# QWTforGithub/CDSegNet

Measured on AMD Instinct MI355X. Metric: points/sec/node (ScanNet ~120k-pt scenes, 1-step), higher is better.
Workload: dtype f16

## Files before the change

### cdsegnet_amd/_lib.py

```python
import ctypes
import os
import threading
from ctypes import POINTER, Structure, c_char_p, c_float, c_int, c_int32, c_int64, c_long, c_size_t, c_uint64, c_void_p

HERE = os.path.dirname(os.path.abspath(__file__))
LIB_PATH = os.path.join(HERE, "libcdseg_hip.so")
LIB_PATH_F16 = os.path.join(HERE, "libcdseg_hip_f16.so")

F32, BF16 = 0, 1
ACT_NONE, ACT_GELU, ACT_SWISH = 0, 1, 2
ORDER_IDS = {"z": 0, "z-trans": 1, "hilbert": 2, "hilbert-trans": 3}
ERRORS = {-1: "CDSEG_ERR_ARG", -2: "CDSEG_ERR_LAUNCH", -3: "CDSEG_ERR_WORKSPACE", -4: "CDSEG_ERR_UNSUPPORTED"}


class CdsegError(RuntimeError):
    pass


class DuplicateVoxelsError(CdsegError):

    def __init__(self, msg, count):
        super().__init__(msg)
        self.count = int(count)

# ... 155 lines not shown
    "cdseg_attn_tail_rr": (c_int, [c_void_p, c_int, c_void_p, c_void_p, c_void_p, c_void_p, c_float, c_void_p, c_void_p,
                                   c_void_p, c_int, c_void_p, c_int, c_long, c_int, c_void_p]),
    "cdseg_cpe_head_rr2": (c_int, [c_void_p, c_int, c_void_p, c_void_p, c_void_p, c_void_p, c_void_p, c_int, c_void_p, c_int,
                                   c_void_p, c_void_p, c_void_p, c_float, c_void_p, c_void_p, c_int, c_long, c_int, c_int, c_void_p]),
    "cdseg_attn_tail_rr2": (c_int, [c_void_p, c_int, c_void_p, c_void_p, c_void_p, c_void_p, c_float, c_void_p, c_void_p,
                                    c_void_p, c_int, c_void_p, c_int, c_void_p, c_int, c_long, c_int, c_void_p, c_size_t, c_void_p]),
    "cdseg_block_scratch_bytes": (c_size_t, [POINTER(BlockDesc), c_long]),
    "cdseg_block_forward": (c_int, [POINTER(BlockDesc), POINTER(BlockIO), c_void_p]),
    "cdseg_layernorm": (c_int, [c_void_p, c_int, c_int, c_void_p, c_void_p, c_float, c_void_p, c_int, c_void_p,
                                c_void_p, c_int, c_int, c_void_p, c_int, c_int, c_long, c_int, c_void_p]),
    "cdseg_attention": (c_int, [c_void_p, c_void_p, c_void_p, c_int, c_int, c_int, c_void_p, c_void_p, c_void_p,
                                c_void_p, c_int, c_int, c_int, c_float, c_void_p, c_int, c_int, c_void_p]),
    "cdseg_attention_ex": (c_int, [c_void_p, c_void_p, c_void_p, c_int, c_int, c_int, c_void_p, c_void_p, c_void_p,
                                   c_void_p, c_int, c_int, c_int, c_float, c_void_p, c_int, c_int, c_int, c_void_p]),
    "cdseg_attention_schedule": (c_long, [c_int, c_int, c_int, c_int, c_void_p, c_long]),
    "cdseg_attention_bwd_ws_bytes": (c_size_t, [c_long, c_int]),
    "cdseg_attention_bwd": (c_int, [c_void_p, c_void_p, c_void_p, c_int, c_int, c_int, c_void_p, c_void_p, c_void_p, c_void_p,
                                    c_int, c_int, c_long, c_int, c_float, c_void_p, c_int, c_void_p, c_void_p, c_void_p,
                                    c_int, c_int, c_int, c_int, c_void_p, c_size_t, c_void_p]),
    "cdseg_layernorm_bwd": (c_int, [c_void_p, c_int, c_void_p, c_float, c_void_p, c_int, c_void_p, c_int, c_int, c_void_p,
                                    c_void_p, c_long, c_int, c_void_p]),
    "cdseg_gelu_bwd": (c_int, [c_void_p, c_void_p, c_void_p, c_long, c_void_p]),
    "cdseg_conv_wgrad": (c_int, [c_void_p, c_int, c_void_p, c_int, c_void_p, c_int, c_long, c_int, c_int, c_void_p, c_void_p,
                                 c_void_p]),
    "cdseg_linear_wgrad": (c_int, [c_void_p, c_int, c_void_p, c_void_p, c_int, c_long, c_int, c_int, c_void_p, c_int, c_void_p,
                                   c_void_p]),
    "cdseg_conv_wgrad16": (c_int, [c_void_p, c_int, c_void_p, c_int, c_void_p, c_int, c_long, c_int, c_int, c_void_p, c_void_p,
                                   c_void_p]),
    "cdseg_linear_wgrad16": (c_int, [c_void_p, c_int, c_void_p, c_void_p, c_int, c_long, c_int, c_int, c_void_p, c_int, c_void_p,
                                     c_void_p]),
# ... 99 lines not shown
```

### cdsegnet_amd/csrc/deep.h

```cpp
#pragma once
#include "common.h"

bool deep_supported(int channels);
int deep_pack(int channels, const void* wl, const void* wqkv, void* head_img, const void* wp, const void* w1, const void* w2,
              void* tail_img, hipStream_t s);
int deep_head(const void* y, int ldy, const void* head_img, const float* bl, const float* lnp_g, const float* lnp_b,
              const float* x, int ldx, float* x_out, int ldxo, const float* colbias, const float* ln1_g, const float* ln1_b,
              float eps, const float* bqkv, void* qkv, int ldqkv, long n, int channels, int qkv_flags, hipStream_t s,
              const float* ypart = nullptr, int ysplits = 1, const float* ybias = nullptr);
struct cdseg_gemm_args;
int gemm_leave_partials(const cdseg_gemm_args* a, int* splits, void* stream);
int deep_tail(const void* o, int ldo, const void* tail_img, const float* bp, const float* ln_g, const float* ln_b, float eps,
              const float* b1, const float* b2, const float* x_in, int ldxi, float* x, int ldx, void* xc, int ldxc, long n,
              int channels, void* ws, size_t ws_bytes, hipStream_t s);
```

### cdsegnet_amd/csrc/gemm.hip

```cpp
#include <cstdlib>

#include <atomic>

#include "common.h"
#include "prof.h"

#ifndef CDSEG_CONV_SQ128_MIN_M
#define CDSEG_CONV_SQ128_MIN_M 8000
#endif
#ifndef CDSEG_CONV_SQ128_MAX_M
#define CDSEG_CONV_SQ128_MAX_M 32768
#endif

namespace {

struct GemmP {
  const void* A;
  const void* W;
  const float* bias;
  const float* scale;
  const float* shift;
  const float* res;
  const float* add_src;
  const int32_t* add_idx;
// ... 11 lines not shown
  int splits;
  int kshift;
  long nbr_sm, nbr_so;
  int gm, gn;
  int xmode;
  int fix;
  const float* colbias;
  const float* ln_pre_g;
  const float* ln_pre_b;
  const float* ln_post_g;
  const float* ln_post_b;
  void* ln_out;
  int ldln, ln_out_dtype;
  float ln_eps;
  int alt;
#ifdef CDSEG_EXPERIMENTS
  int dbg;
#endif
};

struct F32X3 { float v; };
template <typename CT> constexpr bool kIsX3 = false;
template <> constexpr bool kIsX3<F32X3> = true;
typedef _Float16 x3_f16x2_t __attribute__((ext_vector_type(2)));
typedef _Float16 x3_f16x8_t __attribute__((ext_vector_type(8)));

__device__ __forceinline__ void x3_split2(float a, float b, uint32_t& hi, uint32_t& lo) {
  const hw_f32x2_t v = {__builtin_amdgcn_fmed3f(a, -65504.f, 65504.f), __builtin_amdgcn_fmed3f(b, -65504.f, 65504.f)};
  const x3_f16x2_t h = __builtin_convertvector(v, x3_f16x2_t);
  const hw_f32x2_t hf = __builtin_convertvector(h, hw_f32x2_t);
// ... 227 lines not shown
  }
  if (g.ln_post_g) {
    float4 h[MAXG];
    row_layernorm(g.ln_post_g, g.ln_post_b, h);
    if (act_row) {
#pragma unroll
      for (int i = 0; i < MAXG; ++i) {
        const int cg = part + L * i;
        if (cg < groups) store_vec4(g.ln_out, g.ln_out_dtype, m * g.ldln + c0 + 4 * cg, h[i]);
      }
    }
  }
}

__global__ void splitk_epilogue_kernel(GemmP g) {
  const long groups = g.M * (long)(g.N >> 2);
  const long t = (long)blockIdx.x * blockDim.x + threadIdx.x;
  if (t >= groups) return;
  const long m = t / (g.N >> 2);
  const int n = (int)(t - m * (g.N >> 2)) << 2;
  const long stride = g.M * (long)g.N;
  const float* p = g.ws + m * g.N + n;
  float4 v = *reinterpret_cast<const float4*>(p);
  for (int s = 1; s < g.splits; ++s) {
    const float4 u = *reinterpret_cast<const float4*>(p + s * stride);
    v.x += u.x; v.y += u.y; v.z += u.z; v.w += u.w;
  }
  epilogue4(g, m, n, v);
}

__global__ __launch_bounds__(256) void row_finish_kernel(GemmP g) {
  const int lane = threadIdx.x & 63;
  const long m = (long)blockIdx.x * 4 + (threadIdx.x >> 6);
  if (m >= g.M) return;
  const int groups = g.N >> 2;
  const long sstride = g.M * (long)g.N;
  float4 v[2];
#pragma unroll
  for (int i = 0; i < 2; ++i) {
    v[i] = make_float4(0.f, 0.f, 0.f, 0.f);
    if (lane + 64 * i < groups) {
      const float* p = g.ws + m * g.N + 4 * (lane + 64 * i);
      v[i] = *reinterpret_cast<const float4*>(p);
// ... 8 lines not shown

#ifdef CDSEG_GEMM_TIMING
__device__ unsigned long long g_gemm_t[8 * 16384];
extern "C" int cdseg_debug_gemm_timing(unsigned long long* host_dst, size_t count) {
  return hipMemcpyFromSymbol(host_dst, HIP_SYMBOL(g_gemm_t), count * sizeof(unsigned long long)) == hipSuccess ? 0 : -2;
}
__device__ unsigned long long g_gemm_kt[4096 * 16 * 8];
extern "C" int cdseg_debug_gemm_ktiming(unsigned long long* host_dst, size_t count) {
  return hipMemcpyFromSymbol(host_dst, HIP_SYMBOL(g_gemm_kt), count * sizeof(unsigned long long)) == hipSuccess ? 0 : -2;
}
#define KT_STAMP(x) const unsigned long long x = __builtin_readcyclecounter()
#else
#define KT_STAMP(x)
#endif

template <int BN, int BM, bool SQ = false, int AI = 2, int AJ = BN / 32>
__device__ __forceinline__ void tile_epilogue(const GemmP& g, f32x4_t (&acc)[AI][AJ], char* smem, int tid, int lane,
                                              int wm, int wn, long m0, int n0, int zs) {
  constexpr int NT = SQ ? 512 : 4 * BM;
  constexpr int TN = BN / 32;
  constexpr int CLD = BN + 4;
  const int fr = lane & 15, fg = lane >> 4;
  float* Cs = reinterpret_cast<float*>(smem);
  const bool plain = !g.fix && plain_bf16_out(g);
  Cols8 cols;
  if (plain) cols = load_cols8(g, n0 + 8 * (tid % (BN / 8)));
  auto lds_barrier = [] {
    asm volatile("s_waitcnt lgkmcnt(0)" ::: "memory");
    __builtin_amdgcn_s_barrier();
  };
#pragma unroll 1
  for (int hh = 0; hh < BM / 64; ++hh) {
#ifdef CDSEG_GEMM_TIMING
    if (tid == 0 && blockIdx.x < 16384) g_gemm_t[(size_t)blockIdx.x * 8 + 4 + 2 * hh] = __builtin_readcyclecounter();
#endif
    if (hh) lds_barrier();
    int zcol = 0;
    if constexpr (BM > 64) asm volatile("v_mov_b32 %0, 0" : "=v"(zcol));
    if constexpr (SQ) {
// ... 9 lines not shown
      const int rbase = (wm & 1) * 32;
#pragma unroll
      for (int i = 0; i < 2; ++i)
#pragma unroll
        for (int j = 0; j < TN; ++j)
#pragma unroll
          for (int r = 0; r < 4; ++r)
            Cs[(rbase + i * 16 + fg * 4 + r) * CLD + wn * (BN / 2) + j * 16 + fr] = acc[i][j][r];
    }
    lds_barrier();
#ifdef CDSEG_GEMM_TIMING
    if (tid == 0 && blockIdx.x < 16384) g_gemm_t[(size_t)blockIdx.x * 8 + 5 + 2 * hh] = __builtin_readcyclecounter();
#endif
    const long mb = m0 + 64 * hh;
    constexpr int GPR = BN / 4;
    if (g.fix) {
      for (int item = tid; item < 64 * GPR; item += NT) {
        const int row = item / GPR, cg = item % GPR;
        const long m = mb + row;
        const int n = n0 + 4 * cg;
        if (m >= g.M || n >= g.N) continue;
        *reinterpret_cast<float4*>(g.ws + ((long)zs * g.M + m) * g.N + n) =
            *reinterpret_cast<const float4*>(Cs + row * CLD + 4 * cg);
      }
    } else if (BM == 64 && (g.ln_pre_g || g.ln_post_g)) {
      constexpr int MAXG = BN / 16;
      const int row = (tid >> 2) & 63, part = tid & 3;
      const long m = mb + row;
      const int ng = g.N >> 2;
      float4 v[MAXG];
#pragma unroll
      for (int i = 0; i < MAXG; ++i)
        v[i] = (part + 4 * i < ng) ? *reinterpret_cast<const float4*>(Cs + row * CLD + 4 * (part + 4 * i))
                                   : make_float4(0.f, 0.f, 0.f, 0.f);
      finish_row<MAXG>(g, m, m < g.M, part, 4, ng, 0, v);
    } else if (plain) {
      static_assert(NT % (GPR / 2) == 0, "a lane's columns must not change between items");
// ... 259 lines not shown
    if (kc + 1 < kc1) store_tiles();
    __syncthreads();
  }

  if constexpr (kIsX3<CT>) {
#pragma unroll
    for (int i = 0; i < 2; ++i)
#pragma unroll
      for (int j = 0; j < TN; ++j) acc[i][j] += accx[i][j] * (1.0f / 2048.f);
  }
  tile_epilogue<BN, BM>(g, acc, smem, tid, lane, wm, wn, m0, n0, zs);
}

__device__ uint4 g_zero_page[8];

template <int BM, bool GATHER = true, int BN = 128, int NST = 2, bool SQ = false>
struct DmaCfg {
  static constexpr int WAVES = SQ ? 8 : BM / 16, NT = WAVES * 64, BK = 64;
  static constexpr int A_BYTES = BM * 128, W_BYTES = BN * 128;
  static constexpr int A_PW = (BM / 8) / WAVES, W_PW = (BN / 8) / WAVES;
  static constexpr int STAGES = NST * (A_BYTES + W_BYTES);
  static constexpr int ITAB = GATHER ? BM * 27 * 4 : 0;
  static constexpr int LDS = STAGES + ITAB + 1024;
};

template <int BM, bool GATHER, int BN = 128, int NST = 2, bool SQ = false>
__global__ __launch_bounds__(SQ ? 512 : 4 * BM) void gemm_dma_kernel(GemmP g) {
#ifdef CDSEG_GEMM_TIMING
  const unsigned long long rt0 = __builtin_amdgcn_s_memrealtime(), tc0 = __builtin_readcyclecounter();
#endif
  using D = DmaCfg<BM, GATHER, BN, NST, SQ>;
  constexpr int TN = BN / 32;
  constexpr int AI = SQ ? 4 : 2, AJ = TN;
  static_assert(!SQ || (BM == 256 && NST == 2 && GATHER), "SQ: 256-row tiles of 8 waves, two stages, sparse convs");
  extern __shared__ __attribute__((aligned(16))) char smem[];
  char* tail = smem + D::STAGES + D::ITAB;
  int* live = reinterpret_cast<int*>(tail);
  int* glive = reinterpret_cast<int*>(tail + 256);
  unsigned long long* smask = reinterpret_cast<unsigned long long*>(tail + 640);
  int* itab = reinterpret_cast<int*>(smem + D::STAGES);

  const int tid = threadIdx.x;
  const int lane = tid & 63;
  const int wave = __builtin_amdgcn_readfirstlane(tid >> 6);
  const int wm = wave >> 1, wn = wave & 1;
  int mt, sl;
  {
    const int bid = blockIdx.x, slices = g.gn * g.splits;
    if (g.xmode == 1) {
      const int j = bid >> 3;
      mt = j % g.gm;
      sl = (bid & 7) + 8 * (j / g.gm);
      if (sl >= slices) return;
    } else if (g.xmode == 2) {
      const int j = bid >> 3, chunk = (g.gm + 7) >> 3;
      mt = (bid & 7) * chunk + j / slices;
      sl = j % slices;
      if (j / slices >= chunk || mt >= g.gm) return;
    } else {
      mt = bid % g.gm;
      sl = bid / g.gm;
    }
  }
  const int nt = sl % g.gn, zs = sl / g.gn;
  const long m0 = (long)mt * BM;
  const int n0 = nt * BN;
  const long Kw = (long)g.kvol * g.K;

  int nlive = 1;
  if (GATHER) {
    constexpr int OPT = D::NT / BM, PASSES = (27 + OPT - 1) / OPT;
    int* glraw = reinterpret_cast<int*>(tail + 384);
    int* slotmap = reinterpret_cast<int*>(tail + 512);
    const int r = tid % BM, og = tid / BM;
    if (tid < 32) glraw[tid] = 0;
    __syncthreads();
    int idx[PASSES];
#pragma unroll
// ... 23 lines not shown
    __syncthreads();
    nlive = __builtin_amdgcn_readfirstlane(live[0]);
#pragma unroll
    for (int i = 0; i < PASSES; ++i) {
      const int o = og + OPT * i;
      if (o < g.kvol) {
        const int sl2 = slotmap[o];
        if (sl2 >= 0) itab[r * 27 + sl2] = idx[i];
      }
    }
    __syncthreads();
  }
  const int KV = nlive * g.K;
  const int nkc = KV / D::BK;
  const int kshift = g.kshift;
  const int kc0 = (int)(((long)nkc * zs) / g.splits);
  const int kc1 = (int)(((long)nkc * (zs + 1)) / g.splits);

  const int lrow = lane >> 3, slot = lane & 7;
  const bf16_t* a_src[D::A_PW];
  int a_row[D::A_PW];
  int a_chunk[D::A_PW];
  const bf16_t* w_src[D::W_PW];
  int w_chunk[D::W_PW];
#pragma unroll
  for (int i = 0; i < D::A_PW; ++i) {
    const int r = (wave * D::A_PW + i) * 8 + lrow;
    a_row[i] = r;
    a_chunk[i] = slot ^ ((r >> 1) & 7);
    long m = m0 + r;
    if (m >= g.M) m = g.M - 1;
    a_src[i] = (const bf16_t*)g.A + m * g.lda + a_chunk[i] * 8;
// ... 217 lines not shown
  }
#ifdef CDSEG_GEMM_TIMING
  if (lane == 0 && blockIdx.x < 4096 && wave < 16) {
    unsigned long long* d = g_gemm_kt + ((size_t)blockIdx.x * 16 + wave) * 8;
    d[0] = kt_wait; d[1] = kt_bar; d[2] = kt_issue; d[3] = kt_mma; d[4] = (unsigned long long)(kc1 - kc0); d[5] = kt_pro;
    d[6] = (unsigned long long)nlive; d[7] = 1;
  }
#endif
  __syncthreads();
#ifdef CDSEG_EXPERIMENTS
  if (g.dbg & 4) { if (acc[0][0][0] == 12345.678f) ((float*)g.out)[0] = acc[1][1][1]; return; }
#endif
#ifdef CDSEG_GEMM_TIMING
  const unsigned long long tc1 = __builtin_readcyclecounter();
#endif
  tile_epilogue<BN, BM, SQ, AI, AJ>(g, acc, smem, tid, lane, wm, wn, m0, n0, zs);
#ifdef CDSEG_GEMM_TIMING
  if (tid == 0 && blockIdx.x < 16384) {
    unsigned long long* d = g_gemm_t + (size_t)blockIdx.x * 8;
    d[0] = rt0; d[1] = __builtin_amdgcn_s_memrealtime(); d[2] = tc1 - tc0;
    const unsigned long long tend = __builtin_readcyclecounter();
    d[3] = tend - tc1;
    const unsigned long long a0 = d[4], a1 = d[5], b0 = d[6], b1 = d[7];
    d[4] = a1 - a0; d[5] = b0 - a1; d[6] = b1 - b0; d[7] = tend - b1;
  }
#endif
}

thread_local bool tl_leave_partials = false;
thread_local int tl_partial_splits = 1;

template <typename CT, int BN, int NCH, int BM>
constexpr int gemm_smem_bytes() {
  constexpr int ab = (BM + BN) * NCH * 16, c = 64 * (BN + 4) * 4;
  return (ab > c ? ab : c) + 1024;
}


template <typename CT, int NCH, bool GATHER>
int launch_bn(GemmP p, size_t ws_bytes, hipStream_t s) {
  constexpr int BK = NCH * (16 / (int)sizeof(CT));
  static const int split_target = cdseg_knob("CDSEG_GEMM_SPLIT_TARGET", 320);
  static const int split_max = cdseg_knob("CDSEG_GEMM_SPLIT_MAX", 16);
  static const int xmode_env = cdseg_knob("CDSEG_GEMM_XMODE", -1);
  const bool ln = p.ln_pre_g || p.ln_post_g;
// ... 10 lines not shown
  }
  int dma_use_bm = -1;
  if constexpr (NCH == 16 && sizeof(CT) == 2) {
    static const int dma_on0 = cdseg_knob("CDSEG_GEMM_DMA", 1);
    static const int dma_bm0 = cdseg_knob("CDSEG_GEMM_DMA_BM", 0);
    if (dma_on0 && p.N > 64 && (p.K % 64) == 0 && (!GATHER || (p.kshift >= 6 && p.kvol <= 27)) && p.M >= 128) {
      int want = dma_bm0 ? dma_bm0 : ((GATHER || p.M >= 16384 || (p.N >= 1024 && p.M >= 2048)) ? 128 : 64);
      if (ln && p.N <= 128) want = -1;
      if (want > 0) bm = dma_use_bm = want;
    }
  }
  bool sq = false;
  int sq_bn = 256;
  if constexpr (GATHER && NCH == 16 && sizeof(CT) == 2) {
    static const int sq_on = cdseg_knob("CDSEG_CONV_SQ", 1);
    static const int sq_min_m = cdseg_knob("CDSEG_CONV_SQ_MIN_M", 5000);
    static const int sq_min_n = cdseg_knob("CDSEG_CONV_SQ_MIN_N", 256);
    sq = sq_on && dma_use_bm == 128 && p.kvol == 27 && p.N >= sq_min_n && (p.N % 256) == 0 && !ln && p.kshift >= 6 &&
         p.M >= sq_min_m && p.ws && p.vec_ok && !p.out_idx;
    static const int sq128_min_m = cdseg_knob("CDSEG_CONV_SQ128_MIN_M", CDSEG_CONV_SQ128_MIN_M);
    static const int sq128_max_m = cdseg_knob("CDSEG_CONV_SQ128_MAX_M", CDSEG_CONV_SQ128_MAX_M);
    if (!sq && sq_on && sq128_min_m > 0 && dma_use_bm == 128 && p.kvol == 27 && p.N == 128 && !ln && p.kshift >= 6 &&
        p.M >= sq128_min_m && p.M < sq128_max_m && p.vec_ok && !p.out_idx) {
      sq = true;
      sq_bn = 128;
    }
    if (sq) {
      bm = 256;
      p.alt = cdseg_knob("CDSEG_CONV_SQ_ALT", 1);
    }
  }
  const int gm = (int)((p.M + bm - 1) / bm);
  bool wide = false;
  if constexpr (GATHER && NCH == 16 && sizeof(CT) == 2) {
    static const int wide_on = cdseg_knob("CDSEG_CONV_WIDE", 0);
    wide = !sq && wide_on && dma_use_bm == 128 && p.kvol == 27 && p.N >= 256 && (p.N % 256) == 0 && !ln;
  }
  const int bn = wide ? 256 : (sq ? sq_bn : (p.N <= 32 ? 32 : (p.N <= 64 ? 64 : 128)));
  const int gn = (p.N + bn - 1) / bn;
  int splits = 1;
  const long nkc = ((long)p.kvol * p.K + BK - 1) / BK;
  const long blocks = (long)gm * gn;
  const bool can_fix = p.ws && p.vec_ok && !p.out_idx;
  static const int plain_min_nkc = cdseg_knob("CDSEG_GEMM_SPLIT_MIN_NKC", 16);
  if (can_fix && blocks < 256 && nkc >= (GATHER ? 4 : plain_min_nkc)) {
    int smax = (int)(nkc / 2);
    if (smax > split_max) smax = split_max;
    while (smax > 1 && (size_t)smax * p.M * p.N * sizeof(float) > ws_bytes) --smax;
    if (wide || sq) {
      splits = (int)(256 / blocks);
    } else {
      splits = (int)((split_target + blocks - 1) / blocks);
    }
    if (splits > smax) splits = smax;
    if (!wide && !sq)
      for (int c = splits; c <= smax && c < splits + 4; ++c)
        if ((gn * c) % 8 == 0) { splits = c; break; }
    if (splits < 1) splits = 1;
  }
  p.fix = 0;
  if (splits > 1) p.fix = ln ? 2 : 1;
  else if (ln && gn > 1) p.fix = 2;
  if (p.fix) {
    if (!can_fix || (size_t)splits * p.M * p.N * sizeof(float) > ws_bytes) return CDSEG_ERR_WORKSPACE;
    if (p.fix == 2 && p.N > 512) return CDSEG_ERR_UNSUPPORTED;
  }
  p.splits = splits;
  p.gm = gm;
  p.gn = gn;
  const int slices = gn * splits;
  const long wbytes = (long)p.N * p.kvol * p.K * (long)sizeof(CT);
  p.xmode = 0;
  if (sq) p.xmode = gm >= 64 ? 2 : 0;
  else if (slices >= 8 && wbytes >= (1 << 20) && gm > 1) p.xmode = 1;
  else if (GATHER && gm >= 64) p.xmode = 2;
  if (xmode_env >= 0) p.xmode = (xmode_env == 1 && slices < 8) ? 0 : xmode_env;
  unsigned nblk;
  if (p.xmode == 1) nblk = 8u * (unsigned)((slices + 7) / 8) * (unsigned)gm;
  else if (p.xmode == 2) nblk = 8u * (unsigned)((gm + 7) / 8) * (unsigned)slices;
  else nblk = (unsigned)gm * (unsigned)slices;
  const dim3 grid(nblk);
  bool launched = false;
  if constexpr (NCH == 16 && sizeof(CT) == 2) {
    static const int dma_on = cdseg_knob("CDSEG_GEMM_DMA", 1);
    static const int dma_bm = cdseg_knob("CDSEG_GEMM_DMA_BM", 0);
    const bool fused_ln_here = ln && gn == 1 && splits == 1;
    if constexpr (GATHER) {
      if (sq && dma_on && sq_bn == 128) {
        launched = true;
        using Q = DmaCfg<256, true, 128, 2, true>;
        static std::atomic<bool> aq128{false};
        if (!aq128) {
          if (hipFuncSetAttribute((const void*)gemm_dma_kernel<256, true, 128, 2, true>, hipFuncAttributeMaxDynamicSharedMemorySize,
// ... 129 lines not shown
    else hipLaunchKernelGGL((gemm_kernel<CT, 128, NCH, GATHER>), grid, dim3(256), 0, s, p);
  }
  if (hipGetLastError() != hipSuccess) return CDSEG_ERR_LAUNCH;
  if (p.fix == 2) {
    hipLaunchKernelGGL(row_finish_kernel, dim3((unsigned)((p.M + 3) / 4)), dim3(256), 0, s, p);
    if (hipGetLastError() != hipSuccess) return CDSEG_ERR_LAUNCH;
  } else if (p.fix == 1) {
    if (tl_leave_partials && p.vec_ok && p.bias && !p.scale && p.act == CDSEG_ACT_NONE && !p.res && !p.add_src && !p.out2 &&
        !p.out_idx && !p.colbias) {
      tl_partial_splits = p.splits;
      return CDSEG_OK;
    }
    const long groups = p.M * (long)(p.N >> 2);
    hipLaunchKernelGGL(splitk_epilogue_kernel, dim3((unsigned)((groups + 255) / 256)), dim3(256), 0, s, p);
    if (hipGetLastError() != hipSuccess) return CDSEG_ERR_LAUNCH;
  }
  return CDSEG_OK;
}

template <typename CT, bool GATHER>
int launch(const GemmP& p, size_t ws_bytes, hipStream_t s) {
  const long ktot = (long)p.kvol * p.K;
  if (ktot <= 64) {
    if constexpr (sizeof(CT) == 2) return launch_bn<CT, 4, GATHER>(p, ws_bytes, s);
    else return launch_bn<CT, 8, GATHER>(p, ws_bytes, s);
  }
  return launch_bn<CT, 16, GATHER>(p, ws_bytes, s);
}

}
// ... 53 lines not shown
  if (a->compute_dtype == CDSEG_BF16) rc = a->nbr ? launch<bf16_t, true>(p, wsb, s) : launch<bf16_t, false>(p, wsb, s);
  else if (a->compute_dtype == CDSEG_F32) rc = a->nbr ? launch<float, true>(p, wsb, s) : launch<float, false>(p, wsb, s);
  else if (a->compute_dtype == CDSEG_F32X3) rc = a->nbr ? launch<F32X3, true>(p, wsb, s) : launch<F32X3, false>(p, wsb, s);
  if (prof) cdseg_prof_end(tok, s);
  return rc;
}

int gemm_leave_partials(const cdseg_gemm_args* a, int* splits, void* stream) {
  tl_leave_partials = true;
  tl_partial_splits = 1;
  const int rc = cdseg_gemm(a, stream);
  tl_leave_partials = false;
  *splits = tl_partial_splits;
  return rc;
}
```

### cdsegnet_amd/csrc/runtime.hip

```cpp
#include <cstdlib>
#include <cstring>

#include "common.h"
#include "deep.h"

namespace {

inline size_t align_up(size_t v, size_t a) { return (v + a - 1) / a * a; }

struct Carver {
  char* base;
  size_t off, cap;
  void* take(size_t bytes) {
    off = align_up(off, 256);
    void* p = base ? base + off : nullptr;
    off += bytes;
    return p;
  }
};

constexpr int FUSE_LN_MAX_C = 512;
constexpr size_t SPLITK_WS_CAP = (size_t)64 << 20;

inline size_t esz(int dtype) { return dtype == CDSEG_BF16 ? 2 : 4; }
inline int storage_dtype(int dtype) { return dtype == CDSEG_F32X3 ? CDSEG_F32 : dtype; }

struct Layout {
  void *y, *h, *qkv, *o, *u, *y2, *ws, *xs;
  size_t ws_bytes, total;
};

Layout carve(const cdseg_block_desc* d, long n, void* scratch) {
  Carver c{(char*)scratch, 0, 0};
  const size_t e = esz(d->dtype);
  const size_t C = d->channels;
  Layout L;
  L.y = c.take(n * C * e);
  L.h = c.take(n * C * e);
  L.qkv = c.take(n * 3 * C * e);
  L.o = c.take(n * C * e);
  L.u = c.take(n * (size_t)d->hidden * e);
  L.y2 = d->channels > FUSE_LN_MAX_C ? c.take(n * C * 4) : nullptr;
  const long tiles = ((n + 63) / 64) * (((long)C + 127) / 128);
  L.ws_bytes = tiles < 256 ? (size_t)32 * n * (size_t)(3 * C > (size_t)d->hidden ? 3 * C : d->hidden) * 4
                           : (C > 128 ? (size_t)n * C * 4 : 0);
  if (C >= 256 && ((n + 127) / 128) * (((long)C + 255) / 256) < 256) {
    const size_t want = (size_t)8 * n * C * 4;
    if (want > L.ws_bytes) L.ws_bytes = want;
  }
  if (L.ws_bytes > SPLITK_WS_CAP) L.ws_bytes = SPLITK_WS_CAP;
  L.ws = L.ws_bytes ? c.take(L.ws_bytes) : nullptr;
  L.xs = (d->dtype == CDSEG_BF16 && C >= 128 && d->head_img && d->tail_img) ? c.take(n * C * 4) : nullptr;
  L.total = align_up(c.off, 256);
  return L;
}

cdseg_gemm_args base_args(const cdseg_block_desc* d, const Layout& L, long n) {
  cdseg_gemm_args a;
  std::memset(&a, 0, sizeof(a));
  a.M = n;
  a.kvol = 1;
  a.a_dtype = storage_dtype(d->dtype);
  a.compute_dtype = d->dtype;
  a.ws = L.ws;
  a.ws_bytes = L.ws_bytes;
  a.ln_eps = d->ln_eps;
// ... 36 lines not shown
  int rc;
  int attn_flags = d->attn_flags & CDSEG_ATTN_Q_PRESCALED;

  const bool conv_fits = n * 27 * 4 < (1l << 31) && n * (long)C * 2 < (1l << 31) - 65536;
  const bool deep_head_next = cdseg_knob("CDSEG_DEEP_FUSED", 1) != 0 && T == CDSEG_BF16 && (C == 128 || C == 256) &&
                              d->hidden == 4 * C && d->head_img;
  int ysplits = 1;
  const float* ypart = nullptr;
  if (d->cpe_conv_wimg && T == CDSEG_BF16 && (C == 32 || C == 64) && conv_fits) {
    rc = cdseg_subm_conv3(io->xc_in, C, d->cpe_conv_wimg, (const float*)d->cpe_conv_b, io->nbr, n, C, L.y, C, stream);
    if (rc != CDSEG_OK) return rc;
  } else {
    cdseg_gemm_args a = base_args(d, L, n);
    a.A = io->xc_in; a.lda = C; a.W = d->cpe_conv_w; a.bias = d->cpe_conv_b; a.nbr = io->nbr; a.nbr_kmajor = 1; a.kvol = 27;
    a.N = C; a.K = C; a.out = L.y; a.ldo = C; a.out_dtype = T;
    static const bool partials_on = cdseg_knob("CDSEG_CONV_PARTIALS", 1) != 0;
    if (partials_on && deep_head_next && (C == 128 || C == 256) && !io->sat_counter && a.ws && a.bias) {
      if ((rc = gemm_leave_partials(&a, &ysplits, stream)) != CDSEG_OK) return rc;
      if (ysplits > 1) ypart = (const float*)a.ws;
    } else if ((rc = cdseg_gemm(&a, stream)) != CDSEG_OK) {
      return rc;
    }
  }
  static const bool fused_head = cdseg_knob("CDSEG_FUSED_HEAD", 1) != 0;
  static const bool deep_on = cdseg_knob("CDSEG_DEEP_FUSED", 1) != 0;
  static const long deep512_min = cdseg_knob("CDSEG_DEEP512_MIN_ROWS", CDSEG_DEEP512_MIN_ROWS);
  static const bool deep512_split = cdseg_knob("CDSEG_DEEP_SPLIT", 1) != 0;
  const bool deep = deep_on && T == CDSEG_BF16 &&
                    (C == 128 || C == 256 || (C == 512 && (n >= deep512_min || (deep512_split && L.xs)))) && d->hidden == 4 * C;
  const bool head = (fused_head && T == CDSEG_BF16 && (C == 32 || C == 64)) || (deep && d->head_img);
// ... 125 lines not shown
```

### cdsegnet_amd/ops.py

```python
import ctypes
import os
import threading

import torch

from . import _lib
from ._lib import ACT_GELU, ACT_NONE, ACT_SWISH, BF16, F32, GemmArgs, check

__all__ = ["ACT_NONE", "ACT_GELU", "ACT_SWISH", "F32", "BF16"]

LP_DTYPES = {"bf16": torch.bfloat16, "f16": torch.float16}


class _Dtypes:

    def __getitem__(self, dtype):
        if dtype == torch.float32:
            return F32
        if dtype == LP_DTYPES[_lib.active()]:
            return BF16
        raise _lib.CdsegError(f"{dtype} tensors do not belong to the active build of the library ({_lib.active()})")


_DT = _Dtypes()
# ... 504 lines not shown
        a.ln_pre_g, a.ln_pre_b = ln_pre[0].data_ptr(), ln_pre[1].data_ptr()
    else:
        a.ln_pre_g = a.ln_pre_b = None
    if ln_post is not None:
        a.ln_post_g, a.ln_post_b = ln_post[0].data_ptr(), ln_post[1].data_ptr()
        a.ln_out, a.ldln, a.ln_out_dtype = ln_out.data_ptr(), ln_out.stride(0), _DT[ln_out.dtype]
    else:
        a.ln_post_g = a.ln_post_b = a.ln_out = None
    a.ln_eps = float(ln_eps)
    if ((m + 63) >> 6) * ((a.N + 127) >> 7) < 256:
        ws = workspace(min(32 * m * a.N * 4, 64 << 20), out.device)
        a.ws, a.ws_bytes = ws.data_ptr(), ws.numel()
    elif nbr is not None and a.N >= 256 and ((m + 127) >> 7) * ((a.N + 255) >> 8) < 256:
        ws = workspace(min(8 * m * a.N * 4, 64 << 20), out.device)
        a.ws, a.ws_bytes = ws.data_ptr(), ws.numel()
    elif a.N > 128 and (ln_pre is not None or ln_post is not None):
        ws = workspace(m * a.N * 4, out.device)
        a.ws, a.ws_bytes = ws.data_ptr(), ws.numel()
    else:
        a.ws, a.ws_bytes = None, 0
    tok = TIMER.begin("conv" if nbr is not None else "gemm") if TIMER is not None else None
    check(_lib.load().cdseg_gemm(ent[1], _stream()), "gemm")
    if tok is not None:
        TIMER.end(tok, 2.0 * a.M * a.N * a.K * a.kvol)
    return out


FUSED_MLP_CHANNELS = (32, 64, 128)


# ... 655 lines not shown
```

### include/cdseg.h

```cpp
#ifndef CDSEG_H
#define CDSEG_H

#include <stddef.h>
#include <stdint.h>

#ifdef __cplusplus
extern "C" {
#endif

#define CDSEG_OK 0
#define CDSEG_ERR_ARG (-1)
#define CDSEG_ERR_LAUNCH (-2)
#define CDSEG_ERR_WORKSPACE (-3)
#define CDSEG_ERR_UNSUPPORTED (-4)

#define CDSEG_F32 0
#define CDSEG_BF16 1
#define CDSEG_F32X3 2

#define CDSEG_ORDER_Z 0
#define CDSEG_ORDER_Z_TRANS 1
#define CDSEG_ORDER_HILBERT 2
#define CDSEG_ORDER_HILBERT_TRANS 3

// ... 98 lines not shown
int cdseg_layernorm(const void* x, int x_dtype, int ldx, const float* gamma, const float* beta, float eps,
                    const float* res, int ldres, const float* colbias, void* out, int out_dtype, int ldo,
                    void* out2, int out2_dtype, int ldo2, long m, int c, void* stream);

int cdseg_attention(const void* q, const void* k, const void* v, int ldq, int ldk, int ldv, const int32_t* q_gidx,
                    const int32_t* kv_gidx, const int32_t* widx, const int32_t* patch_start, int num_patches,
                    int num_heads, int max_len, float scale, void* out, int ldo, int dtype, void* stream);
#define CDSEG_ATTN_Q_PRESCALED 1
#define CDSEG_ATTN_V_BF16 2
int cdseg_attention_ex(const void* q, const void* k, const void* v, int ldq, int ldk, int ldv, const int32_t* q_gidx,
                       const int32_t* kv_gidx, const int32_t* widx, const int32_t* patch_start, int num_patches,
                       int num_heads, int max_len, float scale, void* out, int ldo, int dtype, int flags, void* stream);

long cdseg_attention_schedule(int num_patches, int num_heads, int max_len, int dtype, int32_t* table, long capacity);

int cdseg_prof_enable(int on);
int cdseg_prof_summary(double* total_ms, long* launches);
#define CDSEG_PROF_ATTENTION 0
#define CDSEG_PROF_CONV 1
#define CDSEG_PROF_CONV_DEEP 2
int cdseg_prof_summary_class(int cls, double* total_ms, long* launches);

int cdseg_segment_max(const void* y, int y_dtype, int ldy, const int32_t* seg_start, long m, int c,
                      const float* scale, const float* shift, int act, float* out, int ldo, void* out2,
                      int out2_dtype, int ldo2, void* stream);
size_t cdseg_pool_fused_img_bytes(int cin, int cout);
int cdseg_pool_fused_pack(const void* w, int cin, int cout, void* wimg, void* stream);
int cdseg_pool_fused(const void* x, int ldx, const void* wimg, const float* bias, const int32_t* seg_start, long m,
                     const float* scale, const float* shift, int act, float* out, int ldo, void* out2, int ldo2,
                     int cin, int cout, void* stream);
// ... 266 lines not shown
```

Measured before the change: 79.95 million.

## Split-K only the tail wave of sparse conv tiles to balance CU rounds

Adds a round planner for the square 256-wide sparse conv GEMM. It takes the last partial wave of output tiles (the remainder after full rounds across CUs) and splits those tiles along K, so the final round fills the device instead of leaving most CUs idle. Whole tiles still run unsplit, and the cut tiles write fp32 partials to a workspace that a split-K epilogue kernel reduces afterwards. A cost model also picks split counts for small grids. Workspace sizing is extended in the runtime and in Python. The cost is an extra reduction launch plus extra workspace traffic and memory.

```diff
diff --git a/cdsegnet_amd/_lib.py b/cdsegnet_amd/_lib.py
--- a/cdsegnet_amd/_lib.py
+++ b/cdsegnet_amd/_lib.py
@@ -193,6 +193,8 @@
     "cdseg_attention_ex": (c_int, [c_void_p, c_void_p, c_void_p, c_int, c_int, c_int, c_void_p, c_void_p, c_void_p,
                                    c_void_p, c_int, c_int, c_int, c_float, c_void_p, c_int, c_int, c_int, c_void_p]),
     "cdseg_attention_schedule": (c_long, [c_int, c_int, c_int, c_int, c_void_p, c_long]),
+    "cdseg_conv_round_plan": (c_long, [c_long, c_int, c_long, c_size_t, c_int, c_int, c_void_p, c_long]),
+    "cdseg_conv_cut_ws_bytes": (c_size_t, [c_long, c_int]),
     "cdseg_attention_bwd_ws_bytes": (c_size_t, [c_long, c_int]),
     "cdseg_attention_bwd": (c_int, [c_void_p, c_void_p, c_void_p, c_int, c_int, c_int, c_void_p, c_void_p, c_void_p, c_void_p,
                                     c_int, c_int, c_long, c_int, c_float, c_void_p, c_int, c_void_p, c_void_p, c_void_p,
diff --git a/cdsegnet_amd/csrc/deep.h b/cdsegnet_amd/csrc/deep.h
--- a/cdsegnet_amd/csrc/deep.h
+++ b/cdsegnet_amd/csrc/deep.h
@@ -10,6 +10,7 @@
               const float* ypart = nullptr, int ysplits = 1, const float* ybias = nullptr);
 struct cdseg_gemm_args;
 int gemm_leave_partials(const cdseg_gemm_args* a, int* splits, void* stream);
+size_t conv_cut_ws_bytes(long M, int channels, int slots);
 int deep_tail(const void* o, int ldo, const void* tail_img, const float* bp, const float* ln_g, const float* ln_b, float eps,
               const float* b1, const float* b2, const float* x_in, int ldxi, float* x, int ldx, void* xc, int ldxc, long n,
               int channels, void* ws, size_t ws_bytes, hipStream_t s);
diff --git a/cdsegnet_amd/csrc/gemm.hip b/cdsegnet_amd/csrc/gemm.hip
--- a/cdsegnet_amd/csrc/gemm.hip
+++ b/cdsegnet_amd/csrc/gemm.hip
@@ -49,6 +49,8 @@
   int ldln, ln_out_dtype;
   float ln_eps;
   int alt;
+  int cut_gm, cut_s, nblk_w;
+  long ws_row0, ws_rows;
 #ifdef CDSEG_EXPERIMENTS
   int dbg;
 #endif
@@ -306,19 +308,19 @@
 }
 
 __global__ void splitk_epilogue_kernel(GemmP g) {
-  const long groups = g.M * (long)(g.N >> 2);
+  const long groups = g.ws_rows * (long)(g.N >> 2);
   const long t = (long)blockIdx.x * blockDim.x + threadIdx.x;
   if (t >= groups) return;
   const long m = t / (g.N >> 2);
   const int n = (int)(t - m * (g.N >> 2)) << 2;
-  const long stride = g.M * (long)g.N;
+  const long stride = g.ws_rows * (long)g.N;
   const float* p = g.ws + m * g.N + n;
   float4 v = *reinterpret_cast<const float4*>(p);
   for (int s = 1; s < g.splits; ++s) {
     const float4 u = *reinterpret_cast<const float4*>(p + s * stride);
     v.x += u.x; v.y += u.y; v.z += u.z; v.w += u.w;
   }
-  epilogue4(g, m, n, v);
+  epilogue4(g, g.ws_row0 + m, n, v);
 }
 
 __global__ __launch_bounds__(256) void row_finish_kernel(GemmP g) {
@@ -357,15 +359,17 @@
 #define KT_STAMP(x)
 #endif
 
-template <int BN, int BM, bool SQ = false, int AI = 2, int AJ = BN / 32>
+template <int BN, int BM, bool SQ = false, int AI = 2, int AJ = BN / 32, bool CUT = false>
 __device__ __forceinline__ void tile_epilogue(const GemmP& g, f32x4_t (&acc)[AI][AJ], char* smem, int tid, int lane,
-                                              int wm, int wn, long m0, int n0, int zs) {
+                                              int wm, int wn, long m0, int n0, int zs, int fix_cut = 0) {
+  const int fix = CUT ? fix_cut : g.fix;
+  const long ws_rows = CUT ? g.ws_rows : g.M, ws_row0 = CUT ? g.ws_row0 : 0;
   constexpr int NT = SQ ? 512 : 4 * BM;
   constexpr int TN = BN / 32;
   constexpr int CLD = BN + 4;
   const int fr = lane & 15, fg = lane >> 4;
   float* Cs = reinterpret_cast<float*>(smem);
-  const bool plain = !g.fix && plain_bf16_out(g);
+  const bool plain = !fix && plain_bf16_out(g);
   Cols8 cols;
   if (plain) cols = load_cols8(g, n0 + 8 * (tid % (BN / 8)));
   auto lds_barrier = [] {
@@ -405,13 +409,13 @@
 #endif
     const long mb = m0 + 64 * hh;
     constexpr int GPR = BN / 4;
-    if (g.fix) {
+    if (fix) {
       for (int item = tid; item < 64 * GPR; item += NT) {
         const int row = item / GPR, cg = item % GPR;
         const long m = mb + row;
         const int n = n0 + 4 * cg;
         if (m >= g.M || n >= g.N) continue;
-        *reinterpret_cast<float4*>(g.ws + ((long)zs * g.M + m) * g.N + n) =
+        *reinterpret_cast<float4*>(g.ws + ((long)zs * ws_rows + (m - ws_row0)) * g.N + n) =
             *reinterpret_cast<const float4*>(Cs + row * CLD + 4 * cg);
       }
     } else if (BM == 64 && (g.ln_pre_g || g.ln_post_g)) {
@@ -701,6 +705,37 @@
 
 __device__ uint4 g_zero_page[8];
 
+template <bool CUT>
+__host__ __device__ __forceinline__ bool dma_block_map(const GemmP& g, int bid, int& mt, int& sl, int& nsp, int& fix) {
+  const int slices = g.gn * g.splits;
+  const int gmw = CUT ? g.gm - g.cut_gm : g.gm;
+  nsp = g.splits;
+  fix = g.fix;
+  if (CUT && g.cut_gm && bid >= g.nblk_w) {
+    const int b2 = bid - g.nblk_w, j = b2 >> 3, r = g.cut_gm * g.gn, chunk = (r + 7) >> 3;
+    const int loc = j / g.cut_s, ct = (b2 & 7) * chunk + loc;
+    if (loc >= chunk || ct >= r) return false;
+    mt = gmw + ct / g.gn;
+    sl = (j - loc * g.cut_s) * g.gn + ct % g.gn;
+    nsp = g.cut_s;
+    fix = 1;
+  } else if (g.xmode == 1) {
+    const int j = bid >> 3;
+    mt = j % gmw;
+    sl = (bid & 7) + 8 * (j / gmw);
+    if (sl >= slices) return false;
+  } else if (g.xmode == 2) {
+    const int j = bid >> 3, chunk = (gmw + 7) >> 3;
+    mt = (bid & 7) * chunk + j / slices;
+    sl = j % slices;
+    if (j / slices >= chunk || mt >= gmw) return false;
+  } else {
+    mt = bid % gmw;
+    sl = bid / gmw;
+  }
+  return true;
+}
+
 template <int BM, bool GATHER = true, int BN = 128, int NST = 2, bool SQ = false>
 struct DmaCfg {
   static constexpr int WAVES = SQ ? 8 : BM / 16, NT = WAVES * 64, BK = 64;
@@ -731,24 +766,9 @@
   const int lane = tid & 63;
   const int wave = __builtin_amdgcn_readfirstlane(tid >> 6);
   const int wm = wave >> 1, wn = wave & 1;
-  int mt, sl;
-  {
-    const int bid = blockIdx.x, slices = g.gn * g.splits;
-    if (g.xmode == 1) {
-      const int j = bid >> 3;
-      mt = j % g.gm;
-      sl = (bid & 7) + 8 * (j / g.gm);
-      if (sl >= slices) return;
-    } else if (g.xmode == 2) {
-      const int j = bid >> 3, chunk = (g.gm + 7) >> 3;
-      mt = (bid & 7) * chunk + j / slices;
-      sl = j % slices;
-      if (j / slices >= chunk || mt >= g.gm) return;
-    } else {
-      mt = bid % g.gm;
-      sl = bid / g.gm;
-    }
-  }
+  constexpr bool CUT = SQ && BN == 256;
+  int mt, sl, nsp, fix;
+  if (!dma_block_map<CUT>(g, blockIdx.x, mt, sl, nsp, fix)) return;
   const int nt = sl % g.gn, zs = sl / g.gn;
   const long m0 = (long)mt * BM;
   const int n0 = nt * BN;
@@ -802,8 +822,8 @@
   const int KV = nlive * g.K;
   const int nkc = KV / D::BK;
   const int kshift = g.kshift;
-  const int kc0 = (int)(((long)nkc * zs) / g.splits);
-  const int kc1 = (int)(((long)nkc * (zs + 1)) / g.splits);
+  const int kc0 = (int)(((long)nkc * zs) / nsp);
+  const int kc1 = (int)(((long)nkc * (zs + 1)) / nsp);
 
   const int lrow = lane >> 3, slot = lane & 7;
   const bf16_t* a_src[D::A_PW];
@@ -1051,7 +1071,7 @@
 #ifdef CDSEG_GEMM_TIMING
   const unsigned long long tc1 = __builtin_readcyclecounter();
 #endif
-  tile_epilogue<BN, BM, SQ, AI, AJ>(g, acc, smem, tid, lane, wm, wn, m0, n0, zs);
+  tile_epilogue<BN, BM, SQ, AI, AJ, CUT>(g, acc, smem, tid, lane, wm, wn, m0, n0, zs, fix);
 #ifdef CDSEG_GEMM_TIMING
   if (tid == 0 && blockIdx.x < 16384) {
     unsigned long long* d = g_gemm_t + (size_t)blockIdx.x * 8;
@@ -1066,6 +1086,80 @@
 
 thread_local bool tl_leave_partials = false;
 thread_local int tl_partial_splits = 1;
+
+constexpr int CONV_CUT_TRAFFIC = 3, CONV_CUT_MIN_GAIN = 5;
+constexpr size_t CONV_CUT_WS_CAP = (size_t)128 << 20;
+constexpr int CONV_SQ_MIN_M = 5000, CONV_SQ_MIN_N = 256;
+struct ConvRoundPlan {
+  int gm, gn, splits;
+  int cut_gm, cut_s;
+};
+ConvRoundPlan conv_round_plan(long M, int N, long nkc, size_t ws_bytes, int slots, int split_max, int cut_on, int force_s) {
+  ConvRoundPlan P;
+  P.gm = (int)((M + 255) / 256);
+  P.gn = (N + 255) / 256;
+  P.splits = 1;
+  P.cut_gm = 0;
+  P.cut_s = 1;
+  const long B = (long)P.gm * P.gn;
+  if (nkc < 4 || slots < 1) return P;
+  int smax = (int)(nkc / 2);
+  if (smax > split_max) smax = split_max;
+  if (B < slots) {
+    int su = smax;
+    while (su > 1 && (size_t)su * M * N * sizeof(float) > ws_bytes) --su;
+    P.splits = (int)(slots / B);
+    if (P.splits > su) P.splits = su;
+    if (P.splits < 1) P.splits = 1;
+    if (cut_on && N > 256 && P.splits == 1 && 2 * B > slots) {
+      long best = 0;
+      int best_s = 1;
+      for (int c = 2; c <= su; ++c) {
+        if (force_s > 0 && c != force_s) continue;
+        if ((size_t)c * M * N * sizeof(float) > CONV_CUT_WS_CAP) break;
+        const long rounds = (B * c + slots - 1) / slots;
+        const long cost = rounds * slots * nkc + (long)CONV_CUT_TRAFFIC * c * c * B;
+        if (best_s == 1 || cost * best_s < best * c) { best = cost; best_s = c; }
+      }
+      if (best_s > 1 && (force_s > 0 || best * 100 < (long)(100 - CONV_CUT_MIN_GAIN) * best_s * slots * nkc)) P.splits = best_s;
+    }
+    return P;
+  }
+  if (!cut_on || slots % P.gn) return P;
+  const long r = B % slots;
+  if (r == 0) return P;
+  const int cut_gm = (int)(r / P.gn);
+  const long cut_rows = M - (long)(P.gm - cut_gm) * 256;
+  int S = (int)(slots / r);
+  if (S > smax) S = smax;
+  while (S > 1 && (size_t)S * cut_rows * N * sizeof(float) > ws_bytes) --S;
+  if (S < 2) return P;
+  P.cut_gm = cut_gm;
+  P.cut_s = S;
+  return P;
+}
+
+unsigned set_cut_tiles(GemmP& p, const ConvRoundPlan& cp) {
+  const int gmw = cp.gm - cp.cut_gm;
+  p.cut_gm = cp.cut_gm;
+  p.cut_s = cp.cut_s;
+  p.ws_row0 = (long)gmw * 256;
+  p.ws_rows = p.M - p.ws_row0;
+  const unsigned whole = p.xmode == 2 ? 8u * (unsigned)((gmw + 7) / 8) * (unsigned)cp.gn : (unsigned)gmw * (unsigned)cp.gn;
+  p.nblk_w = (int)whole;
+  return whole + 8u * (unsigned)((cp.cut_gm * cp.gn + 7) / 8) * (unsigned)cp.cut_s;
+}
+
+int device_cu_count() {
+  static std::atomic<int> cus{0};
+  int c = cus;
+  if (c > 0) return c;
+  int dev = 0;
+  hipDeviceProp_t prop;
+  if (hipGetDevice(&dev) != hipSuccess || hipGetDeviceProperties(&prop, dev) != hipSuccess || prop.multiProcessorCount < 1) return 0;
+  cus = c = prop.multiProcessorCount;
+  return c;
+}
 
 template <typename CT, int BN, int NCH, int BM>
 constexpr int gemm_smem_bytes() {
@@ -1106,8 +1200,8 @@
   int sq_bn = 256;
   if constexpr (GATHER && NCH == 16 && sizeof(CT) == 2) {
     static const int sq_on = cdseg_knob("CDSEG_CONV_SQ", 1);
-    static const int sq_min_m = cdseg_knob("CDSEG_CONV_SQ_MIN_M", 5000);
-    static const int sq_min_n = cdseg_knob("CDSEG_CONV_SQ_MIN_N", 256);
+    static const int sq_min_m = cdseg_knob("CDSEG_CONV_SQ_MIN_M", CONV_SQ_MIN_M);
+    static const int sq_min_n = cdseg_knob("CDSEG_CONV_SQ_MIN_N", CONV_SQ_MIN_N);
     sq = sq_on && dma_use_bm == 128 && p.kvol == 27 && p.N >= sq_min_n && (p.N % 256) == 0 && !ln && p.kshift >= 6 &&
          p.M >= sq_min_m && p.ws && p.vec_ok && !p.out_idx;
     static const int sq128_min_m = cdseg_knob("CDSEG_CONV_SQ128_MIN_M", CDSEG_CONV_SQ128_MIN_M);
@@ -1135,7 +1229,15 @@
   const long blocks = (long)gm * gn;
   const bool can_fix = p.ws && p.vec_ok && !p.out_idx;
   static const int plain_min_nkc = cdseg_knob("CDSEG_GEMM_SPLIT_MIN_NKC", 16);
-  if (can_fix && blocks < 256 && nkc >= (GATHER ? 4 : plain_min_nkc)) {
+  ConvRoundPlan cp{gm, gn, 1, 0, 1};
+  if (sq && sq_bn == 256 && can_fix && xmode_env < 0) {
+    static const int cut_on = cdseg_knob("CDSEG_CONV_CUT", 1);
+    static const int cut_force_s = cdseg_knob("CDSEG_CONV_CUT_S", 0);
+    const int slots = device_cu_count();
+    if (slots < 1) return CDSEG_ERR_LAUNCH;
+    cp = conv_round_plan(p.M, p.N, nkc, ws_bytes, slots, split_max, cut_on, cut_force_s);
+    splits = cp.splits;
+  } else if (can_fix && blocks < 256 && nkc >= (GATHER ? 4 : plain_min_nkc)) {
     int smax = (int)(nkc / 2);
     if (smax > split_max) smax = split_max;
     while (smax > 1 && (size_t)smax * p.M * p.N * sizeof(float) > ws_bytes) --smax;
@@ -1160,15 +1262,20 @@
   p.splits = splits;
   p.gm = gm;
   p.gn = gn;
+  p.cut_gm = p.nblk_w = 0;
+  p.cut_s = 1;
+  p.ws_row0 = 0;
+  p.ws_rows = p.M;
   const int slices = gn * splits;
   const long wbytes = (long)p.N * p.kvol * p.K * (long)sizeof(CT);
   p.xmode = 0;
-  if (sq) p.xmode = gm >= 64 ? 2 : 0;
+  if (sq) p.xmode = gm - cp.cut_gm >= 64 ? 2 : 0;
   else if (slices >= 8 && wbytes >= (1 << 20) && gm > 1) p.xmode = 1;
   else if (GATHER && gm >= 64) p.xmode = 2;
   if (xmode_env >= 0) p.xmode = (xmode_env == 1 && slices < 8) ? 0 : xmode_env;
   unsigned nblk;
-  if (p.xmode == 1) nblk = 8u * (unsigned)((slices + 7) / 8) * (unsigned)gm;
+  if (cp.cut_gm) nblk = set_cut_tiles(p, cp);
+  else if (p.xmode == 1) nblk = 8u * (unsigned)((slices + 7) / 8) * (unsigned)gm;
   else if (p.xmode == 2) nblk = 8u * (unsigned)((gm + 7) / 8) * (unsigned)slices;
   else nblk = (unsigned)gm * (unsigned)slices;
   const dim3 grid(nblk);
@@ -1328,6 +1435,11 @@
     const long groups = p.M * (long)(p.N >> 2);
     hipLaunchKernelGGL(splitk_epilogue_kernel, dim3((unsigned)((groups + 255) / 256)), dim3(256), 0, s, p);
     if (hipGetLastError() != hipSuccess) return CDSEG_ERR_LAUNCH;
+  } else if (p.cut_gm) {
+    p.splits = p.cut_s;
+    const long groups = p.ws_rows * (long)(p.N >> 2);
+    hipLaunchKernelGGL(splitk_epilogue_kernel, dim3((unsigned)((groups + 255) / 256)), dim3(256), 0, s, p);
+    if (hipGetLastError() != hipSuccess) return CDSEG_ERR_LAUNCH;
   }
   return CDSEG_OK;
 }
@@ -1411,3 +1523,41 @@
   *splits = tl_partial_splits;
   return rc;
 }
+
+size_t conv_cut_ws_bytes(long M, int channels, int slots) {
+  if (slots <= 0) slots = device_cu_count();
+  const int C = channels;
+  if (slots < 1 || M < CONV_SQ_MIN_M || C < CONV_SQ_MIN_N || (C % 256) || (C & (C - 1))) return 0;
+  const long nkc = ((long)27 * C + 127) / 128;
+  const ConvRoundPlan P = conv_round_plan(M, C, nkc, CONV_CUT_WS_CAP, slots, 16, 1, 0);
+  size_t want = 0;
+  if (P.cut_gm) want = (size_t)P.cut_s * (size_t)(M - (long)(P.gm - P.cut_gm) * 256) * C * sizeof(float);
+  else if (P.splits > 1 && 2l * P.gm * P.gn > slots) want = (size_t)P.splits * M * C * sizeof(float);
+  return want;
+}
+
+extern "C" size_t cdseg_conv_cut_ws_bytes(long M, int channels) { return M > 0 && channels > 0 ? conv_cut_ws_bytes(M, channels, 0) : 0; }
+
+extern "C" long cdseg_conv_round_plan(long M, int N, long nkc, size_t ws_bytes, int slots, int cut, int32_t* table, long capacity) {
+  if (M <= 0 || N <= 0 || nkc <= 0 || slots <= 0) return CDSEG_ERR_ARG;
+  const ConvRoundPlan cp = conv_round_plan(M, N, nkc, ws_bytes, slots, 16, cut, 0);
+  GemmP p{};
+  p.M = M; p.N = N;
+  p.gm = cp.gm; p.gn = cp.gn; p.splits = cp.splits;
+  p.fix = cp.splits > 1 ? 1 : 0;
+  p.cut_s = 1;
+  p.ws_rows = M;
+  p.xmode = cp.gm - cp.cut_gm >= 64 ? 2 : 0;
+  const int slices = cp.gn * cp.splits;
+  long nblk;
+  if (cp.cut_gm) nblk = set_cut_tiles(p, cp);
+  else if (p.xmode == 2) nblk = 8l * ((cp.gm + 7) / 8) * slices;
+  else nblk = (long)cp.gm * slices;
+  for (long b = 0; b < nblk && b < capacity && table; ++b) {
+    int mt, sl, nsp, fix;
+    int32_t* t = table + 5 * b;
+    if (!dma_block_map<true>(p, (int)b, mt, sl, nsp, fix)) { t[0] = t[1] = t[2] = t[3] = t[4] = -1; continue; }
+    t[0] = mt; t[1] = sl % cp.gn; t[2] = sl / cp.gn; t[3] = nsp; t[4] = fix;
+  }
+  return nblk;
+}
diff --git a/cdsegnet_amd/csrc/runtime.hip b/cdsegnet_amd/csrc/runtime.hip
--- a/cdsegnet_amd/csrc/runtime.hip
+++ b/cdsegnet_amd/csrc/runtime.hip
@@ -27,7 +27,7 @@
 
 struct Layout {
   void *y, *h, *qkv, *o, *u, *y2, *ws, *xs;
-  size_t ws_bytes, total;
+  size_t ws_bytes, conv_ws_bytes, total;
 };
 
 Layout carve(const cdseg_block_desc* d, long n, void* scratch) {
@@ -49,7 +49,12 @@
     if (want > L.ws_bytes) L.ws_bytes = want;
   }
   if (L.ws_bytes > SPLITK_WS_CAP) L.ws_bytes = SPLITK_WS_CAP;
-  L.ws = L.ws_bytes ? c.take(L.ws_bytes) : nullptr;
+  L.conv_ws_bytes = L.ws_bytes;
+  if (d->dtype == CDSEG_BF16 && C >= 256) {
+    const size_t want = conv_cut_ws_bytes(n, (int)C, 0);
+    if (want > L.conv_ws_bytes) L.conv_ws_bytes = want;
+  }
+  L.ws = L.conv_ws_bytes ? c.take(L.conv_ws_bytes) : nullptr;
   L.xs = (d->dtype == CDSEG_BF16 && C >= 128 && d->head_img && d->tail_img) ? c.take(n * C * 4) : nullptr;
   L.total = align_up(c.off, 256);
   return L;
@@ -116,6 +121,7 @@
     cdseg_gemm_args a = base_args(d, L, n);
     a.A = io->xc_in; a.lda = C; a.W = d->cpe_conv_w; a.bias = d->cpe_conv_b; a.nbr = io->nbr; a.nbr_kmajor = 1; a.kvol = 27;
     a.N = C; a.K = C; a.out = L.y; a.ldo = C; a.out_dtype = T;
+    a.ws_bytes = L.conv_ws_bytes;
     static const bool partials_on = cdseg_knob("CDSEG_CONV_PARTIALS", 1) != 0;
     if (partials_on && deep_head_next && (C == 128 || C == 256) && !io->sat_counter && a.ws && a.bias) {
       if ((rc = gemm_leave_partials(&a, &ysplits, stream)) != CDSEG_OK) return rc;
diff --git a/cdsegnet_amd/ops.py b/cdsegnet_amd/ops.py
--- a/cdsegnet_amd/ops.py
+++ b/cdsegnet_amd/ops.py
@@ -542,6 +542,9 @@
     elif nbr is not None and a.N >= 256 and ((m + 127) >> 7) * ((a.N + 255) >> 8) < 256:
         ws = workspace(min(8 * m * a.N * 4, 64 << 20), out.device)
         a.ws, a.ws_bytes = ws.data_ptr(), ws.numel()
+    elif (nbr is not None and a.kvol == 27 and a.N == a.K and a.N >= 256 and is_lp(W.dtype) and out_idx is None and
+          (cut_ws := _lib.load().cdseg_conv_cut_ws_bytes(m, a.N)) > 0):
+        a.ws, a.ws_bytes = workspace(cut_ws, out.device).data_ptr(), cut_ws
     elif a.N > 128 and (ln_pre is not None or ln_post is not None):
         ws = workspace(m * a.N * 4, out.device)
         a.ws, a.ws_bytes = ws.data_ptr(), ws.numel()
diff --git a/include/cdseg.h b/include/cdseg.h
--- a/include/cdseg.h
+++ b/include/cdseg.h
@@ -136,6 +136,9 @@
 
 long cdseg_attention_schedule(int num_patches, int num_heads, int max_len, int dtype, int32_t* table, long capacity);
 
+long cdseg_conv_round_plan(long M, int N, long nkc, size_t ws_bytes, int slots, int cut, int32_t* table, long capacity);
+size_t cdseg_conv_cut_ws_bytes(long M, int channels);
+
 int cdseg_prof_enable(int on);
 int cdseg_prof_summary(double* total_ms, long* launches);
 #define CDSEG_PROF_ATTENTION 0
```

After: 79.11 million. 0.989x the previous value.
